# SJTMusicTeam/MusicGeneration

Hardware: AMD Instinct MI355X
Metric: training events/sec (whole node), REMI seq_len=2048 (higher is better)
Workload: dtype bf16; 1 GPU; cfg2 REMI_EventSeq MusicTransformer V=337 layers=6 d_model=512 seq_len=2048 bf16, fwd+smoothed-CE+bwd+Adam/Noam, dropout 0.2; global_batch=128, per_gpu_batch=128, seq_len=2048, parallelism=dp1, deterministic=True, streams=one stream, whole chip

## Files before the change

### musicgeneration_amd/csrc/rel_attn_bwd.hip

```cpp
#include "rel_attn_common.hpp"

using namespace relattn;

__global__ __launch_bounds__(256) void attn_delta_kernel(const uint16_t* __restrict__ ctx,
                                                         const uint16_t* __restrict__ dctx, const float* __restrict__ lse,
                                                         float* __restrict__ delta, float* __restrict__ nlse2,
                                                         float* __restrict__ ndelta, int B, int L, int d) {
    const int heads = d >> 6;
    const long total = (long)B * L * heads * 8;
    const long gid = (long)blockIdx.x * blockDim.x + threadIdx.x;
    if (gid >= total) return;
    const int sub = (int)(gid & 7);
    const long grp = gid >> 3;
    const int i = (int)(grp % L);
    const int hd = (int)((grp / L) % heads);
    const long row = (grp / ((long)L * heads)) * L + i;
    const size_t off = (size_t)row * d + hd * 64 + sub * 8;
    float a[8], g[8];
    unpack8(*(const u32x4*)(ctx + off), a);
    unpack8(*(const u32x4*)(dctx + off), g);
    float s = 0.f;
#pragma unroll
    for (int k = 0; k < 8; ++k) s += a[k] * g[k];
    s += __shfl_xor(s, 1, 64);
    s += __shfl_xor(s, 2, 64);
    s += __shfl_xor(s, 4, 64);
    if (sub == 0) {
        const size_t si = (size_t)grp;
        delta[si] = s;
        ndelta[si] = -s;
        nlse2[si] = -lse[si] * LOG2E;
    }
}

struct BwdWorkspace { size_t delta, nlse2, ndelta, EfA, EfT, dS, total; };
static BwdWorkspace bwd_workspace(int B, int L, int d) {
    const size_t stat = (((size_t)B * (d / 64) * L * 4) + 255) / 256 * 256, ef = er_frag_bytes(L), nchunk = (size_t)L / 32;
    const size_t dS = 3 * stat + 2 * ef;
    return {0, stat, 2 * stat, 3 * stat, 3 * stat + ef, dS, dS + (size_t)B * (d / 64) * (nchunk * (nchunk + 1) / 2) * 2048};
}

extern "C" size_t mgx_rel_attn_bwd_workspace(int B, int L, int d) { return (B <= 0 || L <= 0 || d <= 0) ? 0 : bwd_workspace(B, L, d).total; }

struct BwdPlan {
    int bg;
    bool dkv64;
    dim3 grid;
    DeTilesPlan de;
};
static int bwd_plan(BwdPlan& p, int B, int L, int d, int parts) {
    p.bg = batch_group(B, L, d, 5);
    MGX_REQUIRE((long)((L + 127) / 128) * (B / p.bg) <= 65535, MGX_ERR_SHAPE, "mgx_rel_attn_bwd: L/128 * batch groups too large");
    p.grid = dim3(p.bg * (d / 64), ((L + 127) / 128) * (B / p.bg));
    MGX_REQUIRE(!((parts & 4) && (parts & 64)), MGX_ERR_SHAPE, "mgx_rel_attn_bwd: parts 4 and 64 both write dk / dv and the dS tiles");
    p.dkv64 = (parts & 4) && L % 128 == 0;
    if (parts & 8) {
        p.de = de_tiles_plan(B, L, d, p.bg);
        MGX_REQUIRE(p.de.grid < (1L << 31), MGX_ERR_SHAPE, "mgx_rel_attn_bwd: grid too large");
    }
    return MGX_OK;
}

extern "C" int mgx_rel_attn_bwd_parts(const uint16_t* qkv, const uint16_t* E, const uint32_t* padbits,
                                      const uint16_t* ctx, const uint16_t* dctx, const float* lse, uint16_t* dqkv,
                                      float* dE, void* workspace, size_t ws_bytes, int B, int L, int d, int M,
                                      int parts, void* stream) {
    MGX_REQUIRE(qkv && E && ctx && dctx && lse && dqkv && dE && workspace, MGX_ERR_NULL, "mgx_rel_attn_bwd: NULL pointer");
    MGX_REQUIRE(B > 0 && L > 0 && d > 0 && d % 64 == 0 && L % 32 == 0 && M >= L, MGX_ERR_SHAPE,
                "mgx_rel_attn_bwd: need d%%64==0, L%%32==0, M>=L (got B=%d L=%d d=%d M=%d)", B, L, d, M);
    const BwdWorkspace ws = bwd_workspace(B, L, d);
    MGX_REQUIRE(ws_bytes >= ws.total && ((uintptr_t)workspace & 255) == 0, MGX_ERR_SHAPE,
                "mgx_rel_attn_bwd: workspace must be 256-byte aligned and >= mgx_rel_attn_bwd_workspace() = %zu bytes (got %zu)", ws.total, ws_bytes);
    MGX_REQUIRE(!((parts & 2) && (parts & 32)), MGX_ERR_SHAPE, "mgx_rel_attn_bwd: parts 2 and 32 both write dq");
    BwdPlan p;
    if (int rc = bwd_plan(p, B, L, d, parts)) return rc;

    char* const base = (char*)workspace;
    float *delta = (float*)(base + ws.delta), *nlse2 = (float*)(base + ws.nlse2), *ndelta = (float*)(base + ws.ndelta);
    u32x4 *EfA = (u32x4*)(base + ws.EfA), *EfT = (u32x4*)(base + ws.EfT);
    uint16_t* dst = (uint16_t*)(base + ws.dS);
    const uint16_t* Er = E + (size_t)(M - L) * 64;
    float* dEr = dE + (size_t)(M - L) * 64;
    if (parts & 1) {
        const long total = (long)B * L * (d / 64) * 8;
        hipLaunchKernelGGL(attn_delta_kernel, dim3((unsigned)((total + 255) / 256)), dim3(256), 0, (hipStream_t)stream, ctx, dctx, lse,
                           delta, nlse2, ndelta, B, L, d);
        launch_er_frag(Er, EfA, EfT, L, (hipStream_t)stream);
    }
    if (p.dkv64) {
        if (int rc = dkv64_launch(qkv, EfA, padbits, dctx, nlse2, ndelta, dqkv, dst, B, L, d, p.bg, stream)) return rc;
    } else if (parts & (4 | 64)) {
        dkv32_launch(qkv, EfA, padbits, dctx, nlse2, ndelta, dqkv, dst, p.grid, L, d, p.bg, stream);
    }
    if (parts & 2) dq_lite_launch(qkv, EfT, dst, dqkv, p.grid, L, d, p.bg, stream);
    if (parts & 32) dq_recompute_launch(qkv, EfA, EfT, padbits, dctx, lse, delta, dqkv, p.grid, L, d, p.bg, stream);
    if (parts & 8)
        if (int rc = de_tiles_launch(qkv, dst, dEr, p.de, L, d, stream)) return rc;
    if (parts & 16) de_recompute_launch(qkv, Er, padbits, dctx, lse, delta, dEr, B, L, d, stream);
    MGX_CHECK_LAUNCH("mgx_rel_attn_bwd");
    return MGX_OK;
}

extern "C" int mgx_rel_attn_bwd(const uint16_t* qkv, const uint16_t* E, const uint32_t* padbits, const uint16_t* ctx,
                                const uint16_t* dctx, const float* lse, uint16_t* dqkv, float* dE, void* workspace,
                                size_t ws_bytes, int B, int L, int d, int M, void* stream) {
    return mgx_rel_attn_bwd_parts(qkv, E, padbits, ctx, dctx, lse, dqkv, dE, workspace, ws_bytes, B, L, d, M, 15, stream);
}
```

### musicgeneration_amd/csrc/rel_attn_common.hpp

```cpp
#pragma once
#include "mgx_common.hpp"

namespace relattn {

constexpr int DH = 64;
constexpr int TILE_BYTES = 32 * DH * 2;
constexpr float LOG2E = 1.4426950408889634f;
constexpr float PAD_NEG = -1.0e9f;

typedef __attribute__((address_space(3))) bf16x4* lds_bf16x4_ptr;
typedef __attribute__((address_space(3))) float* lds_f32_ptr;
typedef __attribute__((address_space(3))) char* lds_char_ptr;
MGX_DEV uint32_t lds_addr_of(const char* p) { return (uint32_t)(uintptr_t)(lds_char_ptr)p; }
MGX_DEV void lds_store_f32(uint32_t addr, float v) { *(lds_f32_ptr)(uintptr_t)addr = v; }

MGX_DEV int crow(int r, int hh) { return (r & 3) + 8 * (r >> 2) + 4 * hh; }

MGX_DEV int imgR_off(int row, int chunk) { return row * 128 + ((chunk ^ ((row >> 1) & 7)) << 4); }
MGX_DEV int imgT_off(int row, int chunk) { return row * 128 + ((chunk ^ (((row >> 1) & 1) << 2)) << 4); }

MGX_DEV bf16x8 frag_R(const char* tile, int row, int hh, int ks) {
    return *(const bf16x8*)(tile + imgR_off(row, 2 * ks + hh));
}

template <int (*IMG_OFF)(int, int)>
MGX_DEV bf16x8 frag_tr(const char* tile, int lane, int s, int ct) {
    const int i = lane & 15, g = lane >> 4, hh = lane >> 5;
    const int rq = i >> 2;
    const int chunk = 4 * ct + 2 * (g & 1) + ((i & 3) >> 1);
    const int byte_in = 8 * (i & 1);
    bf16x8 out;
#pragma unroll
    for (int jq = 0; jq < 2; ++jq) {
        const int row = 16 * s + 8 * jq + 4 * hh + rq;
        bf16x4 t = __builtin_amdgcn_ds_read_tr16_b64_v4bf16((lds_bf16x4_ptr)(tile + IMG_OFF(row, chunk) + byte_in));
        out[4 * jq + 0] = t[0]; out[4 * jq + 1] = t[1]; out[4 * jq + 2] = t[2]; out[4 * jq + 3] = t[3];
    }
    return out;
}
MGX_DEV bf16x8 frag_T(const char* tile, int lane, int s, int ct) { return frag_tr<imgT_off>(tile, lane, s, ct); }
MGX_DEV bf16x8 frag_T_onR(const char* tile, int lane, int s, int ct) { return frag_tr<imgR_off>(tile, lane, s, ct); }

MGX_DEV u32x4 scale8(const u32x4& raw, float sc) {
    float f[8];
    unpack8(raw, f);
#pragma unroll
    for (int k = 0; k < 8; ++k) f[k] *= sc;
    return pack8(f);
}

MGX_DEV bf16x8 acc_to_frag(const f32x16& c, int s) {
    u32x4 w;
    w.x = pack_bf16x2(c[8 * s + 0], c[8 * s + 1]);
    w.y = pack_bf16x2(c[8 * s + 2], c[8 * s + 3]);
    w.z = pack_bf16x2(c[8 * s + 4], c[8 * s + 5]);
    w.w = pack_bf16x2(c[8 * s + 6], c[8 * s + 7]);
    return __builtin_bit_cast(bf16x8, w);
}

MGX_DEV f32x16 mfma(const bf16x8& a, const bf16x8& b, const f32x16& c) {
    return __builtin_amdgcn_mfma_f32_32x32x16_bf16(a, b, c, 0, 0, 0);
}

MGX_DEV f32x16 zero16() {
    f32x16 z;
#pragma unroll
    for (int r = 0; r < 16; ++r) z[r] = 0.f;
    return z;
}

constexpr int BAND_STRIDE = 272;
constexpr int BAND_BYTES = 32 * BAND_STRIDE;
MGX_DEV int band_off(int row, int col) { return row * BAND_STRIDE + col * 4; }
constexpr int BAND_REGION = 16 * BAND_STRIDE;
MGX_DEV int band_rowoff(int a) { return ((a & 3) | ((a >> 3) << 2)) * BAND_STRIDE + ((a >> 2) & 1) * BAND_REGION; }
MGX_DEV void band_store(char* band, const int (&wa0)[16], const int (&wa1)[16], int odd, const f32x16& v) {
    if (odd) {
#pragma unroll
        for (int r = 0; r < 16; ++r) *(float*)(band + wa1[r]) = v[r];
    } else {
#pragma unroll
        for (int r = 0; r < 16; ++r) *(float*)(band + wa0[r]) = v[r];
    }
}

MGX_DEV void dma16(const char* sbase , uint32_t voff, uint32_t lds_wave_base) {
    asm volatile("s_mov_b32 m0, %2\n\ts_nop 0\n\tglobal_load_lds_dwordx4 %1, %0" ::"s"(sbase), "v"(voff), "s"(lds_wave_base) : "memory", "m0");
}
MGX_DEV void dma4(const char* sbase , uint32_t voff, uint32_t lds_wave_base) {
    asm volatile("s_mov_b32 m0, %2\n\ts_nop 0\n\tglobal_load_lds_dword %1, %0" ::"s"(sbase), "v"(voff), "s"(lds_wave_base) : "memory", "m0");
}

MGX_DEV void wave_lds_fence() {
    __builtin_amdgcn_fence(__ATOMIC_RELEASE, "wavefront");
    __builtin_amdgcn_wave_barrier();
    __builtin_amdgcn_fence(__ATOMIC_ACQUIRE, "wavefront");
}

MGX_DEV void store_rows_lds(uint16_t* dst, size_t row_stride, const f32x16& t0, const f32x16& t1, int lane, float sc,
                            char* patch) {
    const int x = lane & 31, hh = lane >> 5;
    wave_lds_fence();
#pragma unroll
    for (int g4 = 0; g4 < 4; ++g4) {
        *(u32x2*)(patch + x * 144 + (8 * g4 + 4 * hh) * 2) =
            u32x2{pack_bf16x2(t0[4 * g4] * sc, t0[4 * g4 + 1] * sc), pack_bf16x2(t0[4 * g4 + 2] * sc, t0[4 * g4 + 3] * sc)};
        *(u32x2*)(patch + x * 144 + (32 + 8 * g4 + 4 * hh) * 2) =
            u32x2{pack_bf16x2(t1[4 * g4] * sc, t1[4 * g4 + 1] * sc), pack_bf16x2(t1[4 * g4 + 2] * sc, t1[4 * g4 + 3] * sc)};
    }
    wave_lds_fence();
    const int rr = lane >> 3, ch = lane & 7;
#pragma unroll
    for (int i = 0; i < 4; ++i) {
        const int row = rr + 8 * i;
        *(u32x4*)(dst + (size_t)row * row_stride + ch * 8) = *(const u32x4*)(patch + row * 144 + ch * 16);
    }
    wave_lds_fence();
}

inline size_t er_frag_bytes(int L) { return (((size_t)L * 64 * 2) + 255) / 256 * 256; }

static __global__ __launch_bounds__(256) void er_frag_kernel(const uint16_t* __restrict__ Er, u32x4* __restrict__ EfA,
                                                             u32x4* __restrict__ EfT, int L) {
    const int n = (L >> 5) * 4 * 64;
    const int gid = blockIdx.x * blockDim.x + threadIdx.x;
    if (gid < n) {
        const int lane = gid & 63, ks = (gid >> 6) & 3, q = gid >> 8;
        const int delta = 32 * q + (lane & 31);
        EfA[gid] = *(const u32x4*)(Er + (size_t)(L - 1 - delta) * 64 + 16 * ks + 8 * (lane >> 5));
    } else if (gid < 2 * n && EfT) {
        const int g = gid - n;
        const int lane = g & 63, ct = (g >> 6) & 1, ks = (g >> 7) & 1, q = g >> 8;
        const int col = 32 * ct + (lane & 31);
        uint16_t v[8];
#pragma unroll
        for (int j = 0; j < 8; ++j) {
            const int delta = 32 * q + 16 * ks + 8 * (lane >> 5) + j;
            v[j] = Er[(size_t)(L - 1 - delta) * 64 + col];
        }
        u32x4 o;
        o.x = v[0] | ((uint32_t)v[1] << 16); o.y = v[2] | ((uint32_t)v[3] << 16);
        o.z = v[4] | ((uint32_t)v[5] << 16); o.w = v[6] | ((uint32_t)v[7] << 16);
        EfT[g] = o;
    }
}

static inline void launch_er_frag(const uint16_t* Er, u32x4* EfA, u32x4* EfT, int L, hipStream_t s) {
    const int n = (L >> 5) * 4 * 64 * (EfT ? 2 : 1);
    hipLaunchKernelGGL(er_frag_kernel, dim3((n + 255) / 256), dim3(256), 0, s, Er, EfA, EfT, L);
}

#ifndef MGX_EXPERIMENTS
#define MGX_EXPERIMENTS 0
#endif

static inline int batch_group(int B, int L, int d, int tensors_per_row) {
    const double per_row = (double)L * d * 2 * tensors_per_row;
    int g = B;
#if MGX_EXPERIMENTS
    static const int forced = [] { const char* e = getenv("MGX_ATTN_BGROUP"); return e ? atoi(e) : 0; }();
    if (forced > 0 && B % forced == 0) return forced;
#endif
    while (g > 1 && (g * per_row > 110e6 || B % g != 0)) --g;
    return g;
}

void dkv32_launch(const uint16_t* qkv, const void* EfA, const uint32_t* padbits, const uint16_t* dctx, const float* nlse2,
                  const float* ndelta, uint16_t* dqkv, uint16_t* dst, dim3 grid, int L, int d, int bg, void* stream);
void dq_lite_launch(const uint16_t* qkv, const void* EfT, const uint16_t* dst, uint16_t* dqkv, dim3 grid, int L, int d, int bg,
                    void* stream);
struct DeTilesPlan { bool dealt ; int rows , ngroups; long wg_per_group, grid; };
DeTilesPlan de_tiles_plan(int B, int L, int d, int bg);
int de_tiles_launch(const uint16_t* qkv, const uint16_t* dst, float* dEr, const DeTilesPlan& p, int L, int d, void* stream);
void dq_recompute_launch(const uint16_t* qkv, const void* EfA, const void* EfT, const uint32_t* padbits, const uint16_t* dctx,
                         const float* lse, const float* delta, uint16_t* dqkv, dim3 grid, int L, int d, int bg, void* stream);
void de_recompute_launch(const uint16_t* qkv, const uint16_t* Er, const uint32_t* padbits, const uint16_t* dctx, const float* lse,
                         const float* delta, float* dEr, int B, int L, int d, void* stream);
int dkv64_launch(const uint16_t* qkv, const void* EfA, const uint32_t* padbits, const uint16_t* dctx, const float* nlse2,
                 const float* ndelta, uint16_t* dqkv, uint16_t* dst, int B, int L, int d, int bg, void* stream);
int fwd64a_launch(const uint16_t* qkv, const void* Ef, const uint32_t* padbits, uint16_t* ctx, float* lse, int B, int L, int d, int bg,
                  void* stream);
int fwd64_launch(const uint16_t* qkv, const void* EfA, const uint32_t* padbits, uint16_t* ctx, float* lse, int B, int L, int d,
                 void* stream);
int fwdpp_launch(const uint16_t* qkv, const void* EfA, const uint32_t* padbits, uint16_t* ctx, float* lse, int B, int L, int d,
                 void* stream);

}
```

### musicgeneration_amd/csrc/rowwise_ops.hip

```cpp
#include <type_traits>
#include "mgx_common.hpp"

__global__ __launch_bounds__(256) void embed_pe_fwd_kernel(
    const int32_t* __restrict__ tok, const float* __restrict__ table, const float* __restrict__ pe,
    uint16_t* __restrict__ out, int rows, int L, int d, int V, float scale, DropCfg dc) {
    const int gpr = d >> 3;
    const long total = (long)rows * gpr;
    for (long g = (long)blockIdx.x * blockDim.x + threadIdx.x; g < total; g += (long)gridDim.x * blockDim.x) {
        const int r = (int)(g / gpr), c = (int)(g % gpr) * 8;
        int t = tok[r];
        t = t < 0 ? 0 : (t >= V ? V - 1 : t);
        const f32x4* tp = (const f32x4*)(table + (size_t)t * d + c);
        const f32x4* pp = (const f32x4*)(pe + (size_t)(r % L) * d + c);
        f32x4 a0 = tp[0], a1 = tp[1], p0 = pp[0], p1 = pp[1];
        float f[8] = {a0.x * scale + p0.x, a0.y * scale + p0.y, a0.z * scale + p0.z, a0.w * scale + p0.w,
                      a1.x * scale + p1.x, a1.y * scale + p1.y, a1.z * scale + p1.z, a1.w * scale + p1.w};
        if (dc.thr16) {
            float m[8];
            drop_mult8(dc, (uint32_t)g, m);
#pragma unroll
            for (int k = 0; k < 8; ++k) f[k] *= m[k];
        }
        *(u32x4*)(out + (size_t)r * d + c) = pack8(f);
    }
}

constexpr int EB_CHUNK = 4096;
constexpr long long EB_BAD_MARK = (long long)0x8000000000000000ull;
template <bool DET>
__global__ __launch_bounds__(256) void embed_bwd_kernel(
    const int32_t* __restrict__ tok, const uint16_t* __restrict__ dout, float* __restrict__ dtable,
    int rows, int d, float scale, DropCfg dc, long long* __restrict__ det) {
    const int v = blockIdx.x;
    const int gpr = d >> 3;
    const int tid = threadIdx.x, lane = tid & 63, w = tid >> 6;
    const int per = ((rows + (int)gridDim.y - 1) / (int)gridDim.y + EB_CHUNK - 1) / EB_CHUNK * EB_CHUNK;
    const int r_lo = blockIdx.y * per, r_hi = min(rows, r_lo + per);
    __shared__ int hits[EB_CHUNK];
    __shared__ int nhit;
    using acc_t = typename std::conditional<DET, long long, float>::type;
    __shared__ acc_t part[3][64][8];
    for (int g0 = 0; g0 < gpr; g0 += 64) {
        const int gi = g0 + lane;
        acc_t acc[8] = {0, 0, 0, 0, 0, 0, 0, 0};
        unsigned bad = 0;
        for (int base = r_lo; base < r_hi; base += EB_CHUNK) {
            if (tid == 0) nhit = 0;
            __syncthreads();
            {
                int tk[EB_CHUNK / 256];
#pragma unroll
                for (int i = 0; i < EB_CHUNK / 256; ++i) {
                    const int r = base + tid + 256 * i;
                    tk[i] = r < r_hi ? tok[r] : -1;
                }
#pragma unroll
                for (int i = 0; i < EB_CHUNK / 256; ++i)
                    if (tk[i] == v) hits[atomicAdd(&nhit, 1)] = base + tid + 256 * i;
            }
            __syncthreads();
            const int n = nhit;
            if (gi < gpr) {
                for (int k0 = w; k0 < n; k0 += 16) {
                    u32x4 raw[4];
                    int rrs[4];
#pragma unroll
                    for (int j = 0; j < 4; ++j) {
                        const int k = k0 + 4 * j;
                        rrs[j] = hits[min(k, n - 1)];
                        raw[j] = *(const u32x4*)(dout + (size_t)rrs[j] * d + gi * 8);
                    }
#pragma unroll
                    for (int j = 0; j < 4; ++j) {
                        if (k0 + 4 * j >= n) break;
                        float f[8];
                        unpack8(raw[j], f);
                        if (dc.thr16) {
                            float m[8];
                            drop_mult8(dc, (uint32_t)((size_t)rrs[j] * gpr + gi), m);
#pragma unroll
                            for (int q = 0; q < 8; ++q) f[q] *= m[q];
                        }
#pragma unroll
                        for (int q = 0; q < 8; ++q) {
                            if (DET) {
                                if (det_representable(f[q])) acc[q] += (acc_t)__float2ll_rn(f[q] * MGX_DET_SCALE);
                                else bad |= 1u << q;
                            } else {
                                acc[q] += (acc_t)f[q];
                            }
                        }
                    }
                }
            }
            __syncthreads();
        }
        if (w > 0) {
#pragma unroll
            for (int q = 0; q < 8; ++q) part[w - 1][lane][q] = (DET && ((bad >> q) & 1u)) ? (acc_t)EB_BAD_MARK : acc[q];
        }
        __syncthreads();
        if (w == 0 && gi < gpr) {
            float* dp = dtable + (size_t)v * d + gi * 8;
#pragma unroll
            for (int q = 0; q < 8; ++q) {
                if (DET) {
                    long long* dq = det + (size_t)v * d + gi * 8 + q;
                    const long long p0 = (long long)part[0][lane][q], p1 = (long long)part[1][lane][q], p2 = (long long)part[2][lane][q];
                    if (((bad >> q) & 1u) || p0 == EB_BAD_MARK || p1 == EB_BAD_MARK || p2 == EB_BAD_MARK) { det_poison(dq); continue; }
                    const long long isum = (long long)acc[q] + p0 + p1 + p2;
                    if (isum != 0) atomicAdd((unsigned long long*)dq, (unsigned long long)isum);
                } else {
                    const float sum = (float)(acc[q] + part[0][lane][q] + part[1][lane][q] + part[2][lane][q]) * scale;
                    if (gridDim.y == 1) dp[q] += sum;
                    else if (sum != 0.f) atomicAdd(dp + q, sum);
                }
            }
        }
        __syncthreads();
    }
}

extern "C" int mgx_embed_pe_fwd(const int32_t* tok, const float* table, const float* pe, uint16_t* out,
                                int B, int L, int d, int V, float p_drop, uint64_t seed, void* stream) {
    MGX_REQUIRE(tok && table && pe && out, MGX_ERR_NULL, "mgx_embed_pe_fwd: NULL pointer");
    MGX_REQUIRE(B > 0 && L > 0 && V > 0 && d > 0 && d % 8 == 0, MGX_ERR_SHAPE,
                "mgx_embed_pe_fwd: need B,L,V>0 and d%%8==0 (got B=%d L=%d d=%d V=%d)", B, L, d, V);
    const long total = (long)B * L * (d / 8);
    int grid = (int)((total + 255) / 256);
    if (grid > 2048) grid = 2048;
    hipLaunchKernelGGL(embed_pe_fwd_kernel, dim3(grid), dim3(256), 0, (hipStream_t)stream, tok, table, pe, out,
                       B * L, L, d, V, sqrtf((float)d), make_drop(p_drop, seed));
    MGX_CHECK_LAUNCH("mgx_embed_pe_fwd");
    return MGX_OK;
}

extern "C" int mgx_embed_bwd(const int32_t* tok, const uint16_t* dout, float* dtable, int B, int L, int d, int V,
                             float p_drop, uint64_t seed, void* stream) {
    MGX_REQUIRE(tok && dout && dtable, MGX_ERR_NULL, "mgx_embed_bwd: NULL pointer");
    MGX_REQUIRE(B > 0 && L > 0 && V > 0 && d > 0 && d % 8 == 0, MGX_ERR_SHAPE,
                "mgx_embed_bwd: need B,L,V>0 and d%%8==0 (got B=%d L=%d d=%d V=%d)", B, L, d, V);
    const long rows = (long)B * L;
    int split = (int)std::min<long>(16, std::max<long>(1, rows / (2 * EB_CHUNK)));
    while (split > 1 && (long)V * split > 8192) --split;
    int rc;
    long long* det = mgx_det_scratch((size_t)V * d, stream, &rc);
    if (rc != MGX_OK) return rc;
    if (det) {
        hipLaunchKernelGGL(embed_bwd_kernel<true>, dim3(V, split), dim3(256), 0, (hipStream_t)stream, tok, dout, dtable, B * L, d,
                           sqrtf((float)d), make_drop(p_drop, seed), det);
        launch_det_fold(det, dtable, (size_t)V * d, sqrtf((float)d), 1, (hipStream_t)stream);
    } else {
        hipLaunchKernelGGL(embed_bwd_kernel<false>, dim3(V, split), dim3(256), 0, (hipStream_t)stream, tok, dout, dtable, B * L, d,
                           sqrtf((float)d), make_drop(p_drop, seed), (long long*)nullptr);
    }
    MGX_CHECK_LAUNCH("mgx_embed_bwd");
    return MGX_OK;
}

__global__ void pad_bitmap_kernel(const int32_t* __restrict__ tok, uint32_t* __restrict__ bits, uint32_t* __restrict__ flag,
                                  int total, int L, int pad) {
    const int i = blockIdx.x * blockDim.x + threadIdx.x;
    const bool p = (i < total) && (tok[i] == pad);
    const unsigned long long m = __ballot(p);
    const int lane = threadIdx.x & 63;
    if (i < total) {
        if (lane == 0) bits[i >> 5] = (uint32_t)m;
        if (lane == 32) bits[i >> 5] = (uint32_t)(m >> 32);
    }
    if (flag && i < total && !p && tok[i - (i % L)] == pad) atomicOr(flag, 1u);
}
extern "C" int mgx_pad_bitmap(const int32_t* tok, uint32_t* bits, uint32_t* flag, int B, int L, int pad, void* stream) {
    MGX_REQUIRE(tok && bits, MGX_ERR_NULL, "mgx_pad_bitmap: NULL pointer");
    MGX_REQUIRE(B > 0 && L > 0 && L % 32 == 0, MGX_ERR_SHAPE, "mgx_pad_bitmap: need L%%32==0 (got L=%d)", L);
    const int total = B * L;
    hipLaunchKernelGGL(pad_bitmap_kernel, dim3((total + 255) / 256), dim3(256), 0, (hipStream_t)stream, tok, bits, flag,
                       total, L, pad);
    MGX_CHECK_LAUNCH("mgx_pad_bitmap");
    return MGX_OK;
}

constexpr int LN_MAXC = 4;
#ifndef MGX_LNF_NT
#define MGX_LNF_NT 2
#endif
#ifndef MGX_LNB_NT
#define MGX_LNB_NT 1
#endif
#define LN_LD(M, p) (((M) & 1) ? __builtin_nontemporal_load(p) : *(p))
#define LN_ST(M, v, p) do { if ((M) & 2) __builtin_nontemporal_store(v, p); else *(p) = (v); } while (0)
#ifndef MGX_LNF_GRID
#define MGX_LNF_GRID 1048576
#endif
#ifndef MGX_LNB_BLOCKS
#define MGX_LNB_BLOCKS 512
#endif

template <int NC>
__global__ __launch_bounds__(256) void add_ln_fwd_kernel(
    const uint16_t* __restrict__ x, const uint16_t* __restrict__ res, const float* __restrict__ gamma,
    const float* __restrict__ beta, uint16_t* __restrict__ out, float* __restrict__ mean_o,
    float* __restrict__ rstd_o, int rows, int d, float eps, DropCfg dc) {
    const int lane = threadIdx.x & 63;
    const int wave = (blockIdx.x * blockDim.x + threadIdx.x) >> 6;
    const int nwave = (gridDim.x * blockDim.x) >> 6;
    const int gpr = d >> 3;
    const float inv_d = 1.f / (float)d;
    for (int r = wave; r < rows; r += nwave) {
        float z[NC][8];
        float s = 0.f;
#pragma unroll
        for (int c = 0; c < NC; ++c) {
            const int col = c * 512 + lane * 8;
            if (col < d) {
                float a[8], b[8];
                unpack8(LN_LD(MGX_LNF_NT, (const u32x4*)(x + (size_t)r * d + col)), a);
                unpack8(LN_LD(MGX_LNF_NT, (const u32x4*)(res + (size_t)r * d + col)), b);
                if (dc.thr16) {
                    float m[8];
                    drop_mult8(dc, (uint32_t)((size_t)r * gpr + (col >> 3)), m);
#pragma unroll
                    for (int k = 0; k < 8; ++k) a[k] *= m[k];
                }
#pragma unroll
                for (int k = 0; k < 8; ++k) { z[c][k] = a[k] + b[k]; s += z[c][k]; }
            } else {
#pragma unroll
                for (int k = 0; k < 8; ++k) z[c][k] = 0.f;
            }
        }
        const float mean = wave_sum(s) / (float)d;
        float q = 0.f;
#pragma unroll
        for (int c = 0; c < NC; ++c) {
            const int col = c * 512 + lane * 8;
            if (col < d) {
#pragma unroll
                for (int k = 0; k < 8; ++k) { const float t = z[c][k] - mean; q += t * t; }
            }
        }
        const float rstd = rsqrtf(wave_sum(q) * inv_d + eps);
        if (lane == 0) { mean_o[r] = mean; rstd_o[r] = rstd; }
#pragma unroll
        for (int c = 0; c < NC; ++c) {
            const int col = c * 512 + lane * 8;
            if (col < d) {
                const f32x4* gp = (const f32x4*)(gamma + col);
                const f32x4* bp = (const f32x4*)(beta + col);
                f32x4 g0 = gp[0], g1 = gp[1], b0 = bp[0], b1 = bp[1];
                const float gg[8] = {g0.x, g0.y, g0.z, g0.w, g1.x, g1.y, g1.z, g1.w};
                const float bb[8] = {b0.x, b0.y, b0.z, b0.w, b1.x, b1.y, b1.z, b1.w};
                float o[8];
#pragma unroll
                for (int k = 0; k < 8; ++k) o[k] = (z[c][k] - mean) * rstd * gg[k] + bb[k];
                LN_ST(MGX_LNF_NT, pack8(o), (u32x4*)(out + (size_t)r * d + col));
            }
        }
    }
}

template <int NC>
__global__ __launch_bounds__(256) void add_ln_bwd_kernel(
    const uint16_t* __restrict__ dout, const uint16_t* __restrict__ x, const uint16_t* __restrict__ res,
    const float* __restrict__ gamma, const float* __restrict__ mean_i, const float* __restrict__ rstd_i,
    uint16_t* __restrict__ dx, uint16_t* __restrict__ dres, float* __restrict__ partial, int rows, int d,
    DropCfg dc, int want_dxsum) {
    const int lane = threadIdx.x & 63;
    const int wid = threadIdx.x >> 6;
    const int wave = (blockIdx.x * blockDim.x + threadIdx.x) >> 6;
    const int nwave = (gridDim.x * blockDim.x) >> 6;
    const int gpr = d >> 3;
    const float inv_d = 1.f / (float)d;
    float ag[NC][8], ab[NC][8], ax[NC][8], gg[NC][8];
#pragma unroll
    for (int c = 0; c < NC; ++c) {
        const int col = c * 512 + lane * 8;
#pragma unroll
        for (int k = 0; k < 8; ++k) {
            ag[c][k] = 0.f; ab[c][k] = 0.f; ax[c][k] = 0.f;
            gg[c][k] = (col < d) ? gamma[col + k] : 0.f;
        }
    }
    u32x4 ra[NC], rb[NC], rd[NC];
    float mean = 0.f, rstd = 0.f;
    auto fetch = [&](int r, u32x4 (&a)[NC], u32x4 (&b)[NC], u32x4 (&dy)[NC], float& mn, float& rs) {
        const int rc = min(r, rows - 1);
        mn = mean_i[rc]; rs = rstd_i[rc];
#pragma unroll
        for (int c = 0; c < NC; ++c) {
            const int col = min(c * 512 + lane * 8, d - 8);
            a[c] = LN_LD(MGX_LNB_NT, (const u32x4*)(x + (size_t)rc * d + col));
            b[c] = LN_LD(MGX_LNB_NT, (const u32x4*)(res + (size_t)rc * d + col));
            dy[c] = LN_LD(MGX_LNB_NT, (const u32x4*)(dout + (size_t)rc * d + col));
        }
    };
    if (wave < rows) fetch(wave, ra, rb, rd, mean, rstd);
    for (int r = wave; r < rows; r += nwave) {
        u32x4 na[NC], nb[NC], nd[NC];
        float nmean, nrstd;
        fetch(r + nwave, na, nb, nd, nmean, nrstd);
        float xh[NC][8], g[NC][8], mult[NC][8];
        float s1 = 0.f, s2 = 0.f;
#pragma unroll
        for (int c = 0; c < NC; ++c) {
            const int col = c * 512 + lane * 8;
            if (col < d) {
                float a[8], b[8], dy[8];
                unpack8(ra[c], a);
                unpack8(rb[c], b);
                unpack8(rd[c], dy);
                if (dc.thr16) drop_mult8(dc, (uint32_t)((size_t)r * gpr + (col >> 3)), mult[c]);
                else {
#pragma unroll
                    for (int k = 0; k < 8; ++k) mult[c][k] = 1.f;
                }
#pragma unroll
                for (int k = 0; k < 8; ++k) {
                    const float z = a[k] * mult[c][k] + b[k];
                    xh[c][k] = (z - mean) * rstd;
                    g[c][k] = dy[k] * gg[c][k];
                    s1 += g[c][k];
                    s2 += g[c][k] * xh[c][k];
                    ag[c][k] += dy[k] * xh[c][k];
                    ab[c][k] += dy[k];
                }
            } else {
#pragma unroll
                for (int k = 0; k < 8; ++k) { xh[c][k] = 0.f; g[c][k] = 0.f; mult[c][k] = 0.f; }
            }
        }
        const float c1 = wave_sum(s1) * inv_d, c2 = wave_sum(s2) * inv_d;
#pragma unroll
        for (int c = 0; c < NC; ++c) {
            const int col = c * 512 + lane * 8;
            if (col < d) {
                float dz[8], dxa[8];
#pragma unroll
                for (int k = 0; k < 8; ++k) {
                    dz[k] = rstd * (g[c][k] - c1 - xh[c][k] * c2);
                    dxa[k] = dz[k] * mult[c][k];
                }
                const u32x4 pz = pack8(dz), px = pack8(dxa);
                LN_ST(MGX_LNB_NT, pz, (u32x4*)(dres + (size_t)r * d + col));
                if (dc.thr16 || dx != dres) LN_ST(MGX_LNB_NT, px, (u32x4*)(dx + (size_t)r * d + col));
                if (want_dxsum) {
                    float q[8];
                    unpack8(px, q);
#pragma unroll
                    for (int k = 0; k < 8; ++k) ax[c][k] += q[k];
                }
            }
        }
#pragma unroll
        for (int c = 0; c < NC; ++c) { ra[c] = na[c]; rb[c] = nb[c]; rd[c] = nd[c]; }
        mean = nmean; rstd = nrstd;
    }
    __shared__ float red[4][512];
    float* prow = partial + (size_t)blockIdx.x * 3 * d;
    const int npass = want_dxsum ? 3 : 2;
    for (int pass = 0; pass < npass; ++pass) {
#pragma unroll
        for (int c = 0; c < NC; ++c) {
            __syncthreads();
#pragma unroll
            for (int k = 0; k < 8; ++k) red[wid][lane * 8 + k] = pass == 0 ? ag[c][k] : (pass == 1 ? ab[c][k] : ax[c][k]);
            __syncthreads();
            for (int j = threadIdx.x; j < 512; j += 256) {
                const int col = c * 512 + j;
                if (col < d) prow[pass * d + col] = red[0][j] + red[1][j] + red[2][j] + red[3][j];
            }
        }
    }
}

__global__ __launch_bounds__(256) void ln_finish_kernel(const float* __restrict__ partial, float* __restrict__ dgamma,
                                                        float* __restrict__ dbeta, float* __restrict__ dxsum, int nblk,
                                                        int d) {
    const int cl = threadIdx.x & 15, part = threadIdx.x >> 4;
    const int idx = blockIdx.x * 16 + cl;
    const int ncol = dxsum ? 3 * d : 2 * d;
    __shared__ float red[16][17];
    float s = 0.f;
    if (idx < ncol) {
        int bb = part;
        for (; bb + 7 * 16 < nblk; bb += 8 * 16) {
            float v[8];
#pragma unroll
            for (int u = 0; u < 8; ++u) v[u] = partial[(size_t)(bb + 16 * u) * 3 * d + idx];
#pragma unroll
            for (int u = 0; u < 8; ++u) s += v[u];
        }
        for (; bb < nblk; bb += 16) s += partial[(size_t)bb * 3 * d + idx];
    }
    red[part][cl] = s;
    __syncthreads();
    if (threadIdx.x < 16 && idx < ncol) {
        float t = 0.f;
#pragma unroll
        for (int r = 0; r < 16; ++r) t += red[r][threadIdx.x];
        float* dst = idx < d ? dgamma + idx : (idx < 2 * d ? dbeta + (idx - d) : dxsum + (idx - 2 * d));
        *dst += t;
    }
}

template <int NC>
static void launch_ln_fwd(const uint16_t* x, const uint16_t* res, const float* gamma, const float* beta,
                          uint16_t* out, float* mean, float* rstd, int rows, int d, float eps, DropCfg dc,
                          hipStream_t s) {
    int grid = (rows + 3) / 4;
    if (grid > MGX_LNF_GRID) grid = MGX_LNF_GRID;
    hipLaunchKernelGGL(add_ln_fwd_kernel<NC>, dim3(grid), dim3(256), 0, s, x, res, gamma, beta, out, mean, rstd,
                       rows, d, eps, dc);
}
constexpr int LN_BWD_BLOCKS = MGX_LNB_BLOCKS;

template <int NC>
static void launch_ln_bwd(const uint16_t* dout, const uint16_t* x, const uint16_t* res, const float* gamma,
                          const float* mean, const float* rstd, uint16_t* dx, uint16_t* dres, float* partial,
                          int grid, int rows, int d, DropCfg dc, int want_dxsum, hipStream_t s) {
    hipLaunchKernelGGL(add_ln_bwd_kernel<NC>, dim3(grid), dim3(256), 0, s, dout, x, res, gamma, mean, rstd, dx,
                       dres, partial, rows, d, dc, want_dxsum);
}

extern "C" int mgx_add_ln_fwd(const uint16_t* x, const uint16_t* res, const float* gamma, const float* beta,
                              uint16_t* out, float* mean, float* rstd, int rows, int d, float eps, float p_drop,
                              uint64_t seed, void* stream) {
    MGX_REQUIRE(x && res && gamma && beta && out && mean && rstd, MGX_ERR_NULL, "mgx_add_ln_fwd: NULL pointer");
    MGX_REQUIRE(rows > 0 && d > 0 && d % 8 == 0 && d <= 512 * LN_MAXC, MGX_ERR_SHAPE,
                "mgx_add_ln_fwd: need d%%8==0 and d<=%d (got rows=%d d=%d)", 512 * LN_MAXC, rows, d);
    const DropCfg dc = make_drop(p_drop, seed);
    const int nc = (d + 511) / 512;
    hipStream_t s = (hipStream_t)stream;
    switch (nc) {
        case 1: launch_ln_fwd<1>(x, res, gamma, beta, out, mean, rstd, rows, d, eps, dc, s); break;
        case 2: launch_ln_fwd<2>(x, res, gamma, beta, out, mean, rstd, rows, d, eps, dc, s); break;
        case 3: launch_ln_fwd<3>(x, res, gamma, beta, out, mean, rstd, rows, d, eps, dc, s); break;
        default: launch_ln_fwd<4>(x, res, gamma, beta, out, mean, rstd, rows, d, eps, dc, s); break;
    }
    MGX_CHECK_LAUNCH("mgx_add_ln_fwd");
    return MGX_OK;
}

extern "C" size_t mgx_add_ln_bwd_workspace(int rows, int d) {
    (void)rows;
    return d > 0 ? (size_t)LN_BWD_BLOCKS * 3 * d * sizeof(float) : 0;
}

extern "C" int mgx_add_ln_bwd(const uint16_t* dout, const uint16_t* x, const uint16_t* res, const float* gamma,
                              const float* mean, const float* rstd, uint16_t* dx, uint16_t* dres, float* dgamma,
                              float* dbeta, float* dxsum, void* workspace, size_t ws_bytes, int rows, int d,
                              float p_drop, uint64_t seed, void* stream) {
    MGX_REQUIRE(dout && x && res && gamma && mean && rstd && dx && dres && dgamma && dbeta && workspace, MGX_ERR_NULL,
                "mgx_add_ln_bwd: NULL pointer");
    MGX_REQUIRE(rows > 0 && d > 0 && d % 8 == 0 && d <= 512 * LN_MAXC, MGX_ERR_SHAPE,
                "mgx_add_ln_bwd: need d%%8==0 and d<=%d (got rows=%d d=%d)", 512 * LN_MAXC, rows, d);
    MGX_REQUIRE(p_drop <= 0.f || dx != dres, MGX_ERR_SHAPE, "mgx_add_ln_bwd: dx may alias dres only when p_drop==0");
    MGX_REQUIRE(ws_bytes >= mgx_add_ln_bwd_workspace(rows, d), MGX_ERR_SHAPE,
                "mgx_add_ln_bwd: workspace must hold mgx_add_ln_bwd_workspace() = %zu bytes (got %zu)",
                mgx_add_ln_bwd_workspace(rows, d), ws_bytes);
    const DropCfg dc = make_drop(p_drop, seed);
    const int nc = (d + 511) / 512;
    hipStream_t s = (hipStream_t)stream;
    int grid = (rows + 3) / 4;
    if (grid > LN_BWD_BLOCKS) grid = LN_BWD_BLOCKS;
    float* partial = (float*)workspace;
    const int wd = dxsum ? 1 : 0;
    switch (nc) {
        case 1: launch_ln_bwd<1>(dout, x, res, gamma, mean, rstd, dx, dres, partial, grid, rows, d, dc, wd, s); break;
        case 2: launch_ln_bwd<2>(dout, x, res, gamma, mean, rstd, dx, dres, partial, grid, rows, d, dc, wd, s); break;
        case 3: launch_ln_bwd<3>(dout, x, res, gamma, mean, rstd, dx, dres, partial, grid, rows, d, dc, wd, s); break;
        default: launch_ln_bwd<4>(dout, x, res, gamma, mean, rstd, dx, dres, partial, grid, rows, d, dc, wd, s); break;
    }
    hipLaunchKernelGGL(ln_finish_kernel, dim3((3 * d + 15) / 16), dim3(256), 0, s, partial, dgamma, dbeta, dxsum, grid, d);
    MGX_CHECK_LAUNCH("mgx_add_ln_bwd");
    return MGX_OK;
}

#ifndef MGX_CE_GRID
#define MGX_CE_GRID 512
#endif
template <int NC>
__global__ __launch_bounds__(1024) void smooth_ce_fwd_kernel(
    const uint16_t* __restrict__ logits, const int32_t* __restrict__ target, float* __restrict__ stats,
    int32_t* __restrict__ argmax_o, float* __restrict__ row_lse, int rows, int V, int ld, float eps_ls, int pad,
    long long* __restrict__ det ) {
    const int lane = threadIdx.x & 63, wid = threadIdx.x >> 6;
    const int wave = (blockIdx.x * blockDim.x + threadIdx.x) >> 6;
    const int nwave = (gridDim.x * blockDim.x) >> 6;
    float loss_acc = 0.f, cnt_acc = 0.f, hit_acc = 0.f, row_acc = 0.f;
    for (int r = wave; r < rows; r += nwave) {
        const uint16_t* lp = logits + (size_t)r * ld;
        const int t = target[r];
        float mx = -INFINITY, sx = 0.f, xt_part = 0.f;
        int am = 0x7fffffff;
        float xr[NC > 0 ? NC : 1][8];
        if (NC > 0) {
#pragma unroll
            for (int c = 0; c < NC; ++c) {
                const int col = 512 * c + 8 * lane;
                if (col < V) unpack8(*(const u32x4*)(lp + col), xr[c]);
#pragma unroll
                for (int k = 0; k < 8; ++k) {
                    if (col + k < V) {
                        sx += xr[c][k];
                        if (xr[c][k] > mx) { mx = xr[c][k]; am = col + k; }
                        if (col + k == t) xt_part = xr[c][k];
                    } else {
                        xr[c][k] = -INFINITY;
                    }
                }
            }
        } else {
            for (int v = lane; v < V; v += 64) {
                const float xv = bf16_to_f32(lp[v]);
                sx += xv;
                if (xv > mx) { mx = xv; am = v; }
            }
        }
#pragma unroll
        for (int o = 32; o > 0; o >>= 1) {
            const float omx = __shfl_xor(mx, o, 64);
            const int oam = __shfl_xor(am, o, 64);
            if (omx > mx || (omx == mx && oam < am)) { mx = omx; am = oam; }
        }
        float se = 0.f;
        if (NC > 0) {
#pragma unroll
            for (int c = 0; c < NC; ++c)
#pragma unroll
                for (int k = 0; k < 8; ++k) se += __expf(xr[c][k] - mx);
        } else {
            for (int v = lane; v < V; v += 64) se += __expf(bf16_to_f32(lp[v]) - mx);
        }
        se = wave_sum(se);
        sx = wave_sum(sx);
        const float lse = mx + __logf(se);
        const float xt_vec = NC > 0 ? wave_sum(xt_part) : 0.f;
        if (lane == 0) {
            const float xt = NC > 0 ? xt_vec : ((t >= 0 && t < V) ? bf16_to_f32(lp[t]) : 0.f);
            row_lse[r] = lse;
            argmax_o[r] = am;
            if (t != pad) {
                loss_acc += lse - (1.f - eps_ls) * xt - (eps_ls / (float)V) * sx;
                cnt_acc += 1.f;
            }
            hit_acc += (am == t) ? 1.f : 0.f;
            row_acc += 1.f;
        }
    }
    __shared__ float red[16][4];
    if (lane == 0) { red[wid][0] = loss_acc; red[wid][1] = cnt_acc; red[wid][2] = hit_acc; red[wid][3] = row_acc; }
    __syncthreads();
    if (threadIdx.x < 4) {
        float v = 0.f;
        for (int i = 0; i < (int)(blockDim.x >> 6); ++i) v += red[i][threadIdx.x];
        if (det) det_add(det + threadIdx.x, v);
        else atomicAdd(stats + threadIdx.x, v);
    }
}

template <bool VEC>
__global__ __launch_bounds__(256) void smooth_ce_bwd_kernel(
    const uint16_t* __restrict__ logits, const int32_t* __restrict__ target, const float* __restrict__ stats,
    const float* __restrict__ row_lse, uint16_t* __restrict__ dlogits, int rows, int V, int ld, float eps_ls,
    int pad, float gscale, const float* __restrict__ gscale_dev) {
    const int lane = threadIdx.x & 63;
    const int wave = (blockIdx.x * blockDim.x + threadIdx.x) >> 6;
    const int nwave = (gridDim.x * blockDim.x) >> 6;
    const float cnt = stats[1];
    const float sc = (gscale_dev ? gscale * gscale_dev[0] : gscale) / cnt;
    const float u = eps_ls / (float)V;
    for (int r = wave; r < rows; r += nwave) {
        const uint16_t* lp = logits + (size_t)r * ld;
        uint16_t* dp = dlogits + (size_t)r * ld;
        const int t = target[r];
        const float lse = row_lse[r];
        const bool keep = (t != pad);
        if (VEC) {
            for (int col = 8 * lane; col < ld; col += 512) {
                float x[8], gv[8];
                if (keep && col < V) unpack8(*(const u32x4*)(lp + col), x);
#pragma unroll
                for (int k = 0; k < 8; ++k) {
                    const int v = col + k;
                    gv[k] = (keep && v < V) ? sc * (__expf(x[k] - lse) - u - ((v == t) ? (1.f - eps_ls) : 0.f)) : 0.f;
                }
                *(u32x4*)(dp + col) = pack8(gv);
            }
            continue;
        }
        for (int v = lane; v < ld; v += 64) {
            float gval = 0.f;
            if (keep && v < V) {
                const float p = __expf(bf16_to_f32(lp[v]) - lse);
                gval = sc * (p - u - ((v == t) ? (1.f - eps_ls) : 0.f));
            }
            dp[v] = f32_to_bf16(gval);
        }
    }
}

extern "C" int mgx_smooth_ce_fwd(const uint16_t* logits, const int32_t* target, float* stats, int32_t* argmax,
                                 float* row_lse, int rows, int V, int ld, float eps_ls, int pad, void* stream) {
    MGX_REQUIRE(logits && target && stats && argmax && row_lse, MGX_ERR_NULL, "mgx_smooth_ce_fwd: NULL pointer");
    MGX_REQUIRE(rows > 0 && V > 0 && ld >= V, MGX_ERR_SHAPE, "mgx_smooth_ce_fwd: need ld>=V (rows=%d V=%d ld=%d)",
                rows, V, ld);
    int grid = (rows + 15) / 16;
    if (grid > MGX_CE_GRID) grid = MGX_CE_GRID;
    int rc;
    long long* det = mgx_det_scratch(4, stream, &rc);
    if (rc != MGX_OK) return rc;
    const bool vec = ld % 8 == 0 && ((uintptr_t)logits & 15) == 0 && V <= 2048;
    const int nc = vec ? (V + 511) / 512 : 0;
#define MGX_CE_FWD(NC) hipLaunchKernelGGL(smooth_ce_fwd_kernel<NC>, dim3(grid), dim3(1024), 0, (hipStream_t)stream, logits, target, stats, \
                                          argmax, row_lse, rows, V, ld, eps_ls, pad, det)
    switch (nc) {
        case 1: MGX_CE_FWD(1); break;
        case 2: MGX_CE_FWD(2); break;
        case 3: MGX_CE_FWD(3); break;
        case 4: MGX_CE_FWD(4); break;
        default: MGX_CE_FWD(0); break;
    }
#undef MGX_CE_FWD
    if (det) launch_det_fold(det, stats, 4, 1.f, 1, (hipStream_t)stream);
    MGX_CHECK_LAUNCH("mgx_smooth_ce_fwd");
    return MGX_OK;
}
extern "C" int mgx_smooth_ce_bwd(const uint16_t* logits, const int32_t* target, const float* stats,
                                 const float* row_lse, uint16_t* dlogits, int rows, int V, int ld, float eps_ls,
                                 int pad, float gscale, const float* gscale_dev, void* stream) {
    MGX_REQUIRE(logits && target && stats && row_lse && dlogits, MGX_ERR_NULL, "mgx_smooth_ce_bwd: NULL pointer");
    MGX_REQUIRE(rows > 0 && V > 0 && ld >= V, MGX_ERR_SHAPE, "mgx_smooth_ce_bwd: need ld>=V (rows=%d V=%d ld=%d)",
                rows, V, ld);
    int grid = (rows + 3) / 4;
    if (grid > 2048) grid = 2048;
    if (ld % 8 == 0 && (((uintptr_t)logits | (uintptr_t)dlogits) & 15) == 0)
        hipLaunchKernelGGL(smooth_ce_bwd_kernel<true>, dim3(grid), dim3(256), 0, (hipStream_t)stream, logits, target, stats,
                           row_lse, dlogits, rows, V, ld, eps_ls, pad, gscale, gscale_dev);
    else
        hipLaunchKernelGGL(smooth_ce_bwd_kernel<false>, dim3(grid), dim3(256), 0, (hipStream_t)stream, logits, target, stats,
                           row_lse, dlogits, rows, V, ld, eps_ls, pad, gscale, gscale_dev);
    MGX_CHECK_LAUNCH("mgx_smooth_ce_bwd");
    return MGX_OK;
}

MGX_DEV float adam_update(float p, float g, float& m, float& v, float lr, float b1, float b2, float eps, float bc1, float bc2s,
                          float gscale) {
    const float gk = g * gscale;
    m = b1 * m + (1.f - b1) * gk;
    v = b2 * v + (1.f - b2) * gk * gk;
    return p - (lr / bc1) * m / (sqrtf(v) / bc2s + eps);
}
MGX_DEV void adam_sweep(float* __restrict__ p, const float* __restrict__ g, float* __restrict__ m, float* __restrict__ v,
                        uint16_t* __restrict__ shadow, size_t n, float lr, float b1, float b2, float eps, float bc1, float bc2s,
                        float gscale) {
    const size_t n4 = n >> 2;
    const size_t stride = (size_t)gridDim.x * blockDim.x;
    for (size_t i = (size_t)blockIdx.x * blockDim.x + threadIdx.x; i < n4; i += stride) {
        f32x4 pp = ((f32x4*)p)[i], gg = ((const f32x4*)g)[i], mm = ((f32x4*)m)[i], vv = ((f32x4*)v)[i];
#pragma unroll
        for (int k = 0; k < 4; ++k) {
            float mk = mm[k], vk = vv[k];
            pp[k] = adam_update(pp[k], gg[k], mk, vk, lr, b1, b2, eps, bc1, bc2s, gscale);
            mm[k] = mk; vv[k] = vk;
        }
        ((f32x4*)p)[i] = pp; ((f32x4*)m)[i] = mm; ((f32x4*)v)[i] = vv;
        if (shadow) {
            u32x2 w = {pack_bf16x2(pp.x, pp.y), pack_bf16x2(pp.z, pp.w)};
            ((u32x2*)shadow)[i] = w;
        }
    }
    const size_t t0 = n4 << 2;
    const size_t i = t0 + (size_t)blockIdx.x * blockDim.x + threadIdx.x;
    if (i < n) {
        float mk = m[i], vk = v[i];
        const float pk = adam_update(p[i], g[i], mk, vk, lr, b1, b2, eps, bc1, bc2s, gscale);
        m[i] = mk; v[i] = vk;
        p[i] = pk;
        if (shadow) shadow[i] = f32_to_bf16(pk);
    }
}
__global__ __launch_bounds__(256) void adam_kernel(float* __restrict__ p, const float* __restrict__ g,
                                                   float* __restrict__ m, float* __restrict__ v,
                                                   uint16_t* __restrict__ shadow, size_t n, float lr, float b1,
                                                   float b2, float eps, float bc1, float bc2s, float gscale) {
    adam_sweep(p, g, m, v, shadow, n, lr, b1, b2, eps, bc1, bc2s, gscale);
}
__global__ __launch_bounds__(256) void adam_clipped_kernel(float* __restrict__ p, const float* __restrict__ g,
                                                           float* __restrict__ m, float* __restrict__ v,
                                                           uint16_t* __restrict__ shadow, size_t n, float lr, float b1,
                                                           float b2, float eps, float bc1, float bc2s,
                                                           const mgx_clip_state* __restrict__ state) {
    const float gscale = state->scale;
    if (state->skipped_last) return;
    adam_sweep(p, g, m, v, shadow, n, lr, b1, b2, eps, bc1, bc2s, gscale);
}

__global__ __launch_bounds__(256) void grad_norm_partial_kernel(const float* __restrict__ g, size_t n, double* __restrict__ workspace) {
    const size_t n4 = n >> 2;
    const size_t stride = (size_t)gridDim.x * blockDim.x;
    double acc = 0.0;
#pragma unroll 4
    for (size_t i = (size_t)blockIdx.x * blockDim.x + threadIdx.x; i < n4; i += stride) {
        const f32x4 gg = ((const f32x4*)g)[i];
#pragma unroll
        for (int k = 0; k < 4; ++k) acc += (double)gg[k] * (double)gg[k];
    }
    const size_t i = (n4 << 2) + (size_t)blockIdx.x * blockDim.x + threadIdx.x;
    if (i < n) acc += (double)g[i] * (double)g[i];
#pragma unroll
    for (int o = 32; o > 0; o >>= 1) acc += __shfl_down(acc, o, 64);
    __shared__ double wsum[4];
    if ((threadIdx.x & 63) == 0) wsum[threadIdx.x >> 6] = acc;
    __syncthreads();
    if (threadIdx.x == 0) workspace[blockIdx.x] = (wsum[0] + wsum[1]) + (wsum[2] + wsum[3]);
}
__global__ __launch_bounds__(256) void grad_norm_finalize_kernel(const double* __restrict__ workspace, int parts, float gscale,
                                                                 float max_norm, mgx_clip_state* __restrict__ state) {
    __shared__ double part[MGX_GRAD_NORM_PARTS];
    for (int i = threadIdx.x; i < parts; i += 256) part[i] = workspace[i];
    __syncthreads();
    if (threadIdx.x != 0) return;
    double sum = 0.0;
#pragma unroll 64
    for (int i = 0; i < parts; ++i) sum += part[i];
    const double norm = sqrt(sum) * fabs((double)gscale);
    state->norm = norm;
    if (isfinite(norm)) {
        const double coef = fmin(1.0, (double)max_norm / (norm + 1e-6));
        state->scale = (float)((double)gscale * coef);
        state->skipped_last = 0u;
        if (coef < 1.0) state->n_clipped += 1;
    } else {
        state->scale = 0.f;
        state->skipped_last = 1u;
        state->n_skipped += 1;
    }
}
__global__ __launch_bounds__(256) void cast_bf16_kernel(const float* __restrict__ p, uint16_t* __restrict__ s, size_t n) {
    const size_t stride = (size_t)gridDim.x * blockDim.x;
    for (size_t i = (size_t)blockIdx.x * blockDim.x + threadIdx.x; i < n; i += stride) s[i] = f32_to_bf16(p[i]);
}

struct AdamLaunch { float bc1, bc2s; unsigned blocks; };
static AdamLaunch adam_launch(size_t n, float beta1, float beta2, int step) {
    size_t blocks = (n / 4 + 255) / 256;
    if (blocks > 2048) blocks = 2048;
    if (blocks < 1) blocks = 1;
    return {1.f - powf(beta1, (float)step), sqrtf(1.f - powf(beta2, (float)step)), (unsigned)blocks};
}
extern "C" int mgx_adam_step(float* p, const float* g, float* m, float* v, uint16_t* shadow, size_t n, float lr,
                             float beta1, float beta2, float eps, int step, float gscale, void* stream) {
    MGX_REQUIRE(p && g && m && v, MGX_ERR_NULL, "mgx_adam_step: NULL pointer");
    MGX_REQUIRE(n > 0 && step >= 1, MGX_ERR_SHAPE, "mgx_adam_step: need n>0 and step>=1 (step=%d)", step);
    MGX_REQUIRE((((uintptr_t)p | (uintptr_t)g | (uintptr_t)m | (uintptr_t)v) & 15) == 0 &&
                    ((uintptr_t)shadow & 7) == 0,
                MGX_ERR_SHAPE, "mgx_adam_step: buffers must be 16-byte aligned");
    const AdamLaunch a = adam_launch(n, beta1, beta2, step);
    hipLaunchKernelGGL(adam_kernel, dim3(a.blocks), dim3(256), 0, (hipStream_t)stream, p, g, m, v, shadow, n,
                       lr, beta1, beta2, eps, a.bc1, a.bc2s, gscale);
    MGX_CHECK_LAUNCH("mgx_adam_step");
    return MGX_OK;
}
static unsigned grad_norm_blocks(size_t n) {
    size_t blocks = (n / 4 + 255) / 256;
    if (blocks > MGX_GRAD_NORM_PARTS) blocks = MGX_GRAD_NORM_PARTS;
    if (blocks < 1) blocks = 1;
    return (unsigned)blocks;
}
extern "C" int mgx_grad_norm(const float* g, size_t n, float gscale, float max_norm, double* workspace, mgx_clip_state* state,
                             void* stream) {
    MGX_REQUIRE(g && workspace && state, MGX_ERR_NULL, "mgx_grad_norm: NULL pointer");
    MGX_REQUIRE(n > 0, MGX_ERR_SHAPE, "mgx_grad_norm: need n>0");
    MGX_REQUIRE(max_norm > 0.f, MGX_ERR_SHAPE, "mgx_grad_norm: max_norm must be > 0 (+inf = never clip), got %g", (double)max_norm);
    MGX_REQUIRE(((uintptr_t)g & 15) == 0 && (((uintptr_t)workspace | (uintptr_t)state) & 7) == 0, MGX_ERR_SHAPE,
                "mgx_grad_norm: g must be 16-byte aligned, workspace and state 8-byte aligned");
    const unsigned blocks = grad_norm_blocks(n);
    hipLaunchKernelGGL(grad_norm_partial_kernel, dim3(blocks), dim3(256), 0, (hipStream_t)stream, g, n, workspace);
    MGX_CHECK_LAUNCH("mgx_grad_norm (partials)");
    hipLaunchKernelGGL(grad_norm_finalize_kernel, dim3(1), dim3(256), 0, (hipStream_t)stream, workspace, (int)blocks, gscale,
                       max_norm, state);
    MGX_CHECK_LAUNCH("mgx_grad_norm (finalize)");
    return MGX_OK;
}
extern "C" int mgx_adam_step_clipped(float* p, const float* g, float* m, float* v, uint16_t* shadow, size_t n, float lr,
                                     float beta1, float beta2, float eps, int step, const mgx_clip_state* state, void* stream) {
    MGX_REQUIRE(p && g && m && v && state, MGX_ERR_NULL, "mgx_adam_step_clipped: NULL pointer");
    MGX_REQUIRE(n > 0 && step >= 1, MGX_ERR_SHAPE, "mgx_adam_step_clipped: need n>0 and step>=1 (step=%d)", step);
    MGX_REQUIRE((((uintptr_t)p | (uintptr_t)g | (uintptr_t)m | (uintptr_t)v) & 15) == 0 &&
                    (((uintptr_t)shadow | (uintptr_t)state) & 7) == 0,
                MGX_ERR_SHAPE, "mgx_adam_step_clipped: buffers must be 16-byte aligned (shadow, state: 8)");
    const AdamLaunch a = adam_launch(n, beta1, beta2, step);
    hipLaunchKernelGGL(adam_clipped_kernel, dim3(a.blocks), dim3(256), 0, (hipStream_t)stream, p, g, m, v, shadow, n,
                       lr, beta1, beta2, eps, a.bc1, a.bc2s, state);
    MGX_CHECK_LAUNCH("mgx_adam_step_clipped");
    return MGX_OK;
}
extern "C" int mgx_cast_bf16(const float* p, uint16_t* shadow, size_t n, void* stream) {
    MGX_REQUIRE(p && shadow, MGX_ERR_NULL, "mgx_cast_bf16: NULL pointer");
    size_t blocks = (n + 255) / 256;
    if (blocks > 2048) blocks = 2048;
    if (blocks < 1) blocks = 1;
    hipLaunchKernelGGL(cast_bf16_kernel, dim3((unsigned)blocks), dim3(256), 0, (hipStream_t)stream, p, shadow, n);
    MGX_CHECK_LAUNCH("mgx_cast_bf16");
    return MGX_OK;
}
```

Measured before the change: 5.250 million events/s.

## Fuse Er fragment prep into attention delta kernel and restructure delta reduction

The backward delta kernel now processes 32 rows per block with batched nontemporal loads, stages the per-head sums in shared memory, and writes delta/nlse2/ndelta in coalesced order. The Er fragment preparation kernel is folded into the same launch as extra blocks, which saves one kernel launch. The embedding forward store is switched to a nontemporal store. This adds shared memory use and more complex indexing. The divergent block roles also add some risk of imbalance.

```diff
diff --git a/musicgeneration_amd/csrc/rel_attn_bwd.hip b/musicgeneration_amd/csrc/rel_attn_bwd.hip
--- a/musicgeneration_amd/csrc/rel_attn_bwd.hip
+++ b/musicgeneration_amd/csrc/rel_attn_bwd.hip
@@ -2,31 +2,52 @@
 
 using namespace relattn;
 
+constexpr int DELTA_ROWS = 32;
 __global__ __launch_bounds__(256) void attn_delta_kernel(const uint16_t* __restrict__ ctx,
                                                          const uint16_t* __restrict__ dctx, const float* __restrict__ lse,
                                                          float* __restrict__ delta, float* __restrict__ nlse2,
-                                                         float* __restrict__ ndelta, int B, int L, int d) {
-    const int heads = d >> 6;
-    const long total = (long)B * L * heads * 8;
-    const long gid = (long)blockIdx.x * blockDim.x + threadIdx.x;
-    if (gid >= total) return;
-    const int sub = (int)(gid & 7);
-    const long grp = gid >> 3;
-    const int i = (int)(grp % L);
-    const int hd = (int)((grp / L) % heads);
-    const long row = (grp / ((long)L * heads)) * L + i;
-    const size_t off = (size_t)row * d + hd * 64 + sub * 8;
-    float a[8], g[8];
-    unpack8(*(const u32x4*)(ctx + off), a);
-    unpack8(*(const u32x4*)(dctx + off), g);
-    float s = 0.f;
+                                                         float* __restrict__ ndelta, int L, int d,
+                                                         const uint16_t* __restrict__ Er, u32x4* __restrict__ EfA,
+                                                         u32x4* __restrict__ EfT, int frag_groups) {
+    extern __shared__ float dsum[];
+    const int heads = d >> 6, cpr = d >> 3;
+    const int tid = threadIdx.x;
+    if ((int)blockIdx.x < frag_groups) {
+        er_frag_unit(Er, EfA, EfT, L, blockIdx.x * 256 + tid);
+        return;
+    }
+    const size_t row0 = (size_t)(blockIdx.x - frag_groups) * DELTA_ROWS;
+    const u32x4* a4 = (const u32x4*)(ctx + row0 * d);
+    const u32x4* g4 = (const u32x4*)(dctx + row0 * d);
+    for (int u0 = 0; u0 < heads; u0 += 8) {
+        u32x4 ra[8], rg[8];
 #pragma unroll
-    for (int k = 0; k < 8; ++k) s += a[k] * g[k];
-    s += __shfl_xor(s, 1, 64);
-    s += __shfl_xor(s, 2, 64);
-    s += __shfl_xor(s, 4, 64);
-    if (sub == 0) {
-        const size_t si = (size_t)grp;
+        for (int j = 0; j < 8; ++j) {
+            const int c = min(u0 + j, heads - 1) * 256 + tid;
+            ra[j] = __builtin_nontemporal_load(a4 + c);
+            rg[j] = __builtin_nontemporal_load(g4 + c);
+        }
+#pragma unroll
+        for (int j = 0; j < 8; ++j) {
+            if (u0 + j >= heads) break;
+            float a[8], g[8];
+            unpack8(ra[j], a);
+            unpack8(rg[j], g);
+            float s = 0.f;
+#pragma unroll
+            for (int k = 0; k < 8; ++k) s += a[k] * g[k];
+            s += __shfl_xor(s, 1, 64);
+            s += __shfl_xor(s, 2, 64);
+            s += __shfl_xor(s, 4, 64);
+            const int c = (u0 + j) * 256 + tid;
+            if ((tid & 7) == 0) dsum[((c % cpr) >> 3) * DELTA_ROWS + c / cpr] = s;
+        }
+    }
+    __syncthreads();
+    const size_t b = row0 / L, i0 = row0 % L;
+    for (int t = tid; t < heads * DELTA_ROWS; t += 256) {
+        const size_t si = (b * heads + (t / DELTA_ROWS)) * L + i0 + (t % DELTA_ROWS);
+        const float s = dsum[t];
         delta[si] = s;
         ndelta[si] = -s;
         nlse2[si] = -lse[si] * LOG2E;
@@ -82,10 +103,11 @@
     const uint16_t* Er = E + (size_t)(M - L) * 64;
     float* dEr = dE + (size_t)(M - L) * 64;
     if (parts & 1) {
-        const long total = (long)B * L * (d / 64) * 8;
-        hipLaunchKernelGGL(attn_delta_kernel, dim3((unsigned)((total + 255) / 256)), dim3(256), 0, (hipStream_t)stream, ctx, dctx, lse,
-                           delta, nlse2, ndelta, B, L, d);
-        launch_er_frag(Er, EfA, EfT, L, (hipStream_t)stream);
+        const int frag_groups = (er_frag_units(L, true) + 255) / 256;
+        const long groups = (long)B * L / DELTA_ROWS + frag_groups;
+        MGX_REQUIRE(groups < (1L << 31), MGX_ERR_SHAPE, "mgx_rel_attn_bwd: grid too large");
+        hipLaunchKernelGGL(attn_delta_kernel, dim3((unsigned)groups), dim3(256), (d / 64) * DELTA_ROWS * sizeof(float), (hipStream_t)stream,
+                           ctx, dctx, lse, delta, nlse2, ndelta, L, d, Er, EfA, EfT, frag_groups);
     }
     if (p.dkv64) {
         if (int rc = dkv64_launch(qkv, EfA, padbits, dctx, nlse2, ndelta, dqkv, dst, B, L, d, p.bg, stream)) return rc;
diff --git a/musicgeneration_amd/csrc/rel_attn_common.hpp b/musicgeneration_amd/csrc/rel_attn_common.hpp
--- a/musicgeneration_amd/csrc/rel_attn_common.hpp
+++ b/musicgeneration_amd/csrc/rel_attn_common.hpp
@@ -120,10 +120,10 @@
 
 inline size_t er_frag_bytes(int L) { return (((size_t)L * 64 * 2) + 255) / 256 * 256; }
 
-static __global__ __launch_bounds__(256) void er_frag_kernel(const uint16_t* __restrict__ Er, u32x4* __restrict__ EfA,
-                                                             u32x4* __restrict__ EfT, int L) {
+inline int er_frag_units(int L, bool both) { return (L >> 5) * 4 * 64 * (both ? 2 : 1); }
+
+MGX_DEV void er_frag_unit(const uint16_t* __restrict__ Er, u32x4* __restrict__ EfA, u32x4* __restrict__ EfT, int L, int gid) {
     const int n = (L >> 5) * 4 * 64;
-    const int gid = blockIdx.x * blockDim.x + threadIdx.x;
     if (gid < n) {
         const int lane = gid & 63, ks = (gid >> 6) & 3, q = gid >> 8;
         const int delta = 32 * q + (lane & 31);
@@ -145,9 +145,13 @@
     }
 }
 
+static __global__ __launch_bounds__(256) void er_frag_kernel(const uint16_t* __restrict__ Er, u32x4* __restrict__ EfA,
+                                                             u32x4* __restrict__ EfT, int L) {
+    er_frag_unit(Er, EfA, EfT, L, blockIdx.x * blockDim.x + threadIdx.x);
+}
+
 static inline void launch_er_frag(const uint16_t* Er, u32x4* EfA, u32x4* EfT, int L, hipStream_t s) {
-    const int n = (L >> 5) * 4 * 64 * (EfT ? 2 : 1);
-    hipLaunchKernelGGL(er_frag_kernel, dim3((n + 255) / 256), dim3(256), 0, s, Er, EfA, EfT, L);
+    hipLaunchKernelGGL(er_frag_kernel, dim3((er_frag_units(L, EfT != nullptr) + 255) / 256), dim3(256), 0, s, Er, EfA, EfT, L);
 }
 
 #ifndef MGX_EXPERIMENTS
diff --git a/musicgeneration_amd/csrc/rowwise_ops.hip b/musicgeneration_amd/csrc/rowwise_ops.hip
--- a/musicgeneration_amd/csrc/rowwise_ops.hip
+++ b/musicgeneration_amd/csrc/rowwise_ops.hip
@@ -21,7 +21,7 @@
 #pragma unroll
             for (int k = 0; k < 8; ++k) f[k] *= m[k];
         }
-        *(u32x4*)(out + (size_t)r * d + c) = pack8(f);
+        __builtin_nontemporal_store(pack8(f), (u32x4*)(out + (size_t)r * d + c));
     }
 }
 
```

Result: no change. 5.265 million events/s (median of 6 runs) (+0.3%).
